# umautobots/LONER

Measured on AMD Instinct MI355X. Metric: training rays/sec, higher is better.
Workload: dtype f32

## Files before the change

### loner_amd/csrc/lnr_table_reduce.hip

```cpp
#include "lnr_density_api.h"
#include <cstdlib>

#define LNR_SLAB_GROUPS 16
__device__ __forceinline__ void slab_fold_block(const float* __restrict__ slabs, int n_slabs, int n_mlp, float* __restrict__ grad, int overwrite, int block) {
    __shared__ float part[LNR_SLAB_GROUPS][64];
    const int px = threadIdx.x & 63, gy = threadIdx.x >> 6;
    const int i = block * 64 + px;
    const int per = (n_slabs + LNR_SLAB_GROUPS - 1) / LNR_SLAB_GROUPS;
    int b = gy * per;
    const int b_end = min(n_slabs, b + per);
    float s0 = 0.0f, s1 = 0.0f, s2 = 0.0f, s3 = 0.0f;
    if (i < n_mlp) {
        for (; b + 3 < b_end; b += 4) {
            s0 += slabs[(size_t)b * n_mlp + i]; s1 += slabs[(size_t)(b + 1) * n_mlp + i];
            s2 += slabs[(size_t)(b + 2) * n_mlp + i]; s3 += slabs[(size_t)(b + 3) * n_mlp + i];
        }
        for (; b < b_end; ++b) s0 += slabs[(size_t)b * n_mlp + i];
    }
    part[gy][px] = (s0 + s1) + (s2 + s3);
    __syncthreads();
    if (gy == 0 && i < n_mlp) {
        float s = 0.0f;
#pragma unroll
        for (int k = 0; k < LNR_SLAB_GROUPS; ++k) s += part[k][px];
        grad[i] = overwrite ? s : grad[i] + s;
    }
}
__global__ void __launch_bounds__(64 * LNR_SLAB_GROUPS)
reduce_slabs_kernel(const float* __restrict__ slabs, int n_slabs, int n_mlp, float* __restrict__ grad, int overwrite) {
    slab_fold_block(slabs, n_slabs, n_mlp, grad, overwrite, (int)blockIdx.x);
}

template <int PAIR>
__device__ __forceinline__ void reduce_one(long long* acc, uint2 r, uint32_t base) {
    if (PAIR) {
        uint32_t pi; float v0, v1;
        lnr_unpack_pair(r, pi, v0, v1);
        unsigned long long* a = reinterpret_cast<unsigned long long*>(acc) + 2 * pi;
        if (__builtin_expect(__builtin_fmaxf(__builtin_fabsf(v0), __builtin_fabsf(v1)) < 256.0f, 1)) {
            atomicAdd(a, (unsigned long long)lnr_to_fix_small(v0));
            atomicAdd(a + 1, (unsigned long long)lnr_to_fix_small(v1));
        } else {
            atomicAdd(a, (unsigned long long)lnr_to_fix(v0));
            atomicAdd(a + 1, (unsigned long long)lnr_to_fix(v1));
        }
    } else {
        const float v = __uint_as_float(r.y);
        if (v != 0.0f) atomicAdd(reinterpret_cast<unsigned long long*>(&acc[r.x - base]), (unsigned long long)lnr_to_fix(v));
    }
}
__device__ __forceinline__ void reduce_xpair(long long* acc, const LnrXRec& r) {
    uint32_t pi, t; float a0, a1, fx;
    lnr_unpack_xpair(r, pi, t, a0, a1, fx);
    const uint32_t pj = pi ^ ((2u << t) - 1u);
    long long q[4];
    lnr_xpair_fix(a0, a1, fx, q);
    unsigned long long* a = reinterpret_cast<unsigned long long*>(acc);
    atomicAdd(a + 2 * pi, (unsigned long long)q[0]);
    atomicAdd(a + 2 * pi + 1, (unsigned long long)q[1]);
    atomicAdd(a + 2 * pj, (unsigned long long)q[2]);
    atomicAdd(a + 2 * pj + 1, (unsigned long long)q[3]);
}

#ifdef LNR_PHASE_TIMING
__device__ unsigned long long lnr_reduce_phase_cycles[LNR_N_PHASES];
#endif
#define RED_SLICE (1 << LNR_SLICE_SHIFT)

typedef uint32_t red_u32x3 __attribute__((ext_vector_type(3), aligned(4)));
typedef uint32_t red_u32x4 __attribute__((ext_vector_type(4)));
__device__ __forceinline__ LnrXRec load_xrec_stream(const char* p) {
    const red_u32x3 v = __builtin_nontemporal_load(reinterpret_cast<const red_u32x3*>(p));
    LnrXRec r; r.a = v.x; r.b = v.y; r.c = v.z;
    return r;
}
__device__ __forceinline__ uint4 load_rec2_stream(const uint4* p) {
    const red_u32x4 v = __builtin_nontemporal_load(reinterpret_cast<const red_u32x4*>(p));
    return make_uint4(v.x, v.y, v.z, v.w);
}

template <int PAIR, int RED_U>
__device__ __forceinline__ void reduce_regions(long long* acc, const int* __restrict__ wave_counts, const char* __restrict__ wave_regions, int n_regions,
                                               uint32_t region_bytes, bool xp, uint32_t base, int lane) {
    for (int r0 = 0; r0 < n_regions; r0 += 64) {
        const int nq = min(64, n_regions - r0);
        const int my_n = lane < nq ? wave_counts[r0 + lane] : 0;
        const char* round_regions = wave_regions + (size_t)r0 * region_bytes;
        if (xp) {
            LnrXRec cur[RED_U][2], nxt[RED_U][2];
            auto loadx = [&](int q0, LnrXRec out[RED_U][2]) {
#pragma unroll
                for (int u = 0; u < RED_U; ++u) {
                    const int q = q0 + u < nq ? q0 + u : nq - 1;
                    const int n = __builtin_amdgcn_readlane(my_n, q);
                    const char* rg = round_regions + (size_t)q * region_bytes;
                    out[u][0] = load_xrec_stream(rg + (lane < n ? lane : 0) * 12);
                    out[u][1] = load_xrec_stream(rg + (lane + 64 < n ? lane + 64 : 0) * 12);
                }
            };
            loadx(0, nxt);
            for (int q0 = 0; q0 < nq; q0 += RED_U) {
#pragma unroll
                for (int u = 0; u < RED_U; ++u) { cur[u][0] = nxt[u][0]; cur[u][1] = nxt[u][1]; }
                if (q0 + RED_U < nq) loadx(q0 + RED_U, nxt);
#pragma unroll
                for (int u = 0; u < RED_U; ++u) {
                    const int n = q0 + u < nq ? __builtin_amdgcn_readlane(my_n, q0 + u < 64 ? q0 + u : 63) : 0;
                    if (lane < n) reduce_xpair(acc, cur[u][0]);
                    if (lane + 64 < n) reduce_xpair(acc, cur[u][1]);
                }
            }
            unsigned long long more = __ballot(my_n > 128);
            while (more) {
                const int q = __builtin_ctzll(more);
                more &= more - 1ull;
                const int n = __builtin_amdgcn_readlane(my_n, q);
                const char* rg = round_regions + (size_t)q * region_bytes;
                for (int off = 128; off < n; off += 64 * 4) {
                    LnrXRec r[4];
#pragma unroll
                    for (int u = 0; u < 4; ++u) { const int k = off + 64 * u + lane; r[u] = load_xrec_stream(rg + (size_t)(k < n ? k : n - 1) * 12); }
#pragma unroll
                    for (int u = 0; u < 4; ++u) if (off + 64 * u + lane < n) reduce_xpair(acc, r[u]);
                }
            }
            continue;
        }
        uint4 cur[RED_U], nxt[RED_U];
        auto load4 = [&](int q0, uint4 out[RED_U]) {
#pragma unroll
            for (int u = 0; u < RED_U; ++u) {
                const int q = q0 + u < nq ? q0 + u : nq - 1;
                const int n = __builtin_amdgcn_readlane(my_n, q);
                out[u] = load_rec2_stream(reinterpret_cast<const uint4*>(round_regions + (size_t)q * region_bytes) + (2 * lane < n ? lane : 0));
            }
        };
        load4(0, nxt);
        for (int q0 = 0; q0 < nq; q0 += RED_U) {
#pragma unroll
            for (int u = 0; u < RED_U; ++u) cur[u] = nxt[u];
            if (q0 + RED_U < nq) load4(q0 + RED_U, nxt);
#pragma unroll
            for (int u = 0; u < RED_U; ++u) {
                const int n = q0 + u < nq ? __builtin_amdgcn_readlane(my_n, q0 + u < 64 ? q0 + u : 63) : 0;
                if (2 * lane < n) reduce_one<PAIR>(acc, make_uint2(cur[u].x, cur[u].y), base);
                if (2 * lane + 1 < n) reduce_one<PAIR>(acc, make_uint2(cur[u].z, cur[u].w), base);
            }
        }
        unsigned long long more = __ballot(my_n > 128);
        while (more) {
            const int q = __builtin_ctzll(more);
            more &= more - 1ull;
            const int n = __builtin_amdgcn_readlane(my_n, q);
            const uint2* rg = reinterpret_cast<const uint2*>(round_regions + (size_t)q * region_bytes);
            for (int off = 128; off < n; off += 128 * 4) {
                uint4 r[4];
#pragma unroll
                for (int u = 0; u < 4; ++u) { const int k = off + 128 * u + 2 * lane; r[u] = load_rec2_stream(reinterpret_cast<const uint4*>(rg) + (k < n ? k : 0) / 2); }
#pragma unroll
                for (int u = 0; u < 4; ++u) {
                    const int k = off + 128 * u + 2 * lane;
                    if (k < n) reduce_one<PAIR>(acc, make_uint2(r[u].x, r[u].y), base);
                    if (k + 1 < n) reduce_one<PAIR>(acc, make_uint2(r[u].z, r[u].w), base);
                }
            }
        }
    }
}

struct RedLevel { uint64_t lo, hi; };
__device__ __forceinline__ RedLevel red_level(const LnrNetSpec& spec, int l) {
    RedLevel r;
    r.lo = (uint64_t)spec.level_offset[l] * spec.n_features;
    r.hi = r.lo + (uint64_t)spec.level_size[l] * spec.n_features;
    return r;
}

template <int PAIR, int RED_U, int MINW>
__global__ void __launch_bounds__(1024, MINW)
table_grad_reduce_split_kernel(const LnrNetSpec spec, const void* __restrict__ regions_v, const RegionPlan plan, const int* __restrict__ counts, int bpg,
                               int maxo, long long* __restrict__ ovf) {
    extern __shared__ long long acc[];
    constexpr int slice = RED_SLICE, shift = LNR_SLICE_SHIFT;
    int b = blockIdx.x, l = 0, span = 0;
    int64_t my_ovf = 0;
    RedLevel lv;
    for (;; ++l) {
        lv = red_level(spec, l);
        span = (int)(((lv.hi - 1) >> shift) - (lv.lo >> shift)) + 1;
        const int n = plan.split[l] > 1 ? span * plan.split[l] : 0;
        if (b < n) break;
        b -= n;
        my_ovf += (int64_t)(lv.hi - lv.lo);
    }
    const int parts = plan.split[l], local = b / parts, part = b % parts;
    const uint32_t base = ((uint32_t)(lv.lo >> shift) + (uint32_t)local) << shift;
    const uint32_t region_bytes = plan.bytes[l];
    if (region_bytes == 0u) return;
#pragma unroll
    for (int i = threadIdx.x; i < slice; i += 1024) acc[i] = 0ll;
    __syncthreads();
    const int lane = threadIdx.x & 63, wave = __builtin_amdgcn_readfirstlane(threadIdx.x >> 6);
    const int per_part = (bpg + parts - 1) / parts, part_first = part * per_part, part_n = min(per_part, bpg - part_first);
    const int per_wave = (part_n + 15) / 16, first = part_first + wave * per_wave, n_regions = min(per_wave, part_first + part_n - first);
    if (n_regions > 0)
        reduce_regions<PAIR, RED_U>(acc, counts + ((size_t)l * maxo + local) * bpg + first,
                                    reinterpret_cast<const char*>(regions_v) + plan.off[l] + ((size_t)local * bpg + first) * (size_t)region_bytes, n_regions,
                                    region_bytes, PAIR && plan.xp[l] != 0, base, lane);
    __syncthreads();
#pragma unroll
    for (int k = 0; k < slice / 1024; ++k) {
        const int i = threadIdx.x + k * 1024;
        const uint64_t gi = (uint64_t)base + i;
        const long long q = acc[i];
        if (q != 0ll && gi >= lv.lo && gi < lv.hi) atomicAdd(reinterpret_cast<unsigned long long*>(ovf + my_ovf + (int64_t)(gi - lv.lo)), (unsigned long long)q);
    }
}

template <int PAIR, int RED_U, int MINW>
__global__ void __launch_bounds__(1024, MINW)
table_grad_reduce2_kernel(const LnrNetSpec spec, const void* __restrict__ regions_v, const RegionPlan plan, const int* __restrict__ counts, int bpg,
                          int maxo, long long* __restrict__ ovf, const int* __restrict__ ovf_flag, int epoch, float* __restrict__ grad_table,
                          int64_t n_table_floats, int overwrite, const float* __restrict__ slabs, int n_slabs, int n_mlp, float* __restrict__ grad_mlp) {
    extern __shared__ long long acc[];
    const int slab_blocks = slabs != nullptr ? (n_mlp + 63) / 64 : 0;
    const int owner_blocks = (int)gridDim.x - slab_blocks;
    if ((int)blockIdx.x >= owner_blocks) {
        slab_fold_block(slabs, n_slabs, n_mlp, grad_mlp, overwrite, (int)blockIdx.x - owner_blocks);
        return;
    }
    const int o = owner_blocks - 1 - (int)blockIdx.x;
    constexpr int slice = RED_SLICE, shift = LNR_SLICE_SHIFT;
    const uint32_t base = (uint32_t)o << shift;
    PHASE_INIT();
#pragma unroll
    for (int i = threadIdx.x; i < slice; i += 1024) acc[i] = 0ll;
    __syncthreads();
    PHASE(0);
    const int lane = threadIdx.x & 63, wave = __builtin_amdgcn_readfirstlane(threadIdx.x >> 6);
    constexpr int nwaves = 16;
    int64_t ovf_off = 0;
    for (int l = 0; l < spec.n_levels; ++l) {
        const RedLevel lv = red_level(spec, l);
        const uint64_t lo = lv.lo, hi = lv.hi;
        const int64_t my_ovf = ovf_off;
        ovf_off += (int64_t)(hi - lo);
        if (hi <= base || lo >= (uint64_t)base + slice) continue;
        if (plan.split[l] > 1 || ovf_flag[l] == epoch) {
            long long v[slice / 1024];
#pragma unroll
            for (int k = 0; k < slice / 1024; ++k) {
                const uint64_t gi = (uint64_t)base + threadIdx.x + k * 1024;
                v[k] = (gi >= lo && gi < hi) ? ovf[my_ovf + (int64_t)(gi - lo)] : 0ll;
            }
#pragma unroll
            for (int k = 0; k < slice / 1024; ++k) {
                if (v[k] != 0ll) {
                    acc[threadIdx.x + k * 1024] += v[k];
                    ovf[my_ovf + (int64_t)((uint64_t)base + threadIdx.x + k * 1024 - lo)] = 0ll;
                }
            }
            __syncthreads();
            PHASE(1);
        }
        const int local = o - (int)(lo >> shift);
        if (local < 0 || local >= maxo) continue;
        const uint32_t region_bytes = plan.bytes[l];
        if (region_bytes == 0u || plan.split[l] > 1) continue;
        const int per_wave = (bpg + nwaves - 1) / nwaves;
        const int first = wave * per_wave;
        const int n_regions = min(per_wave, bpg - first);
        if (n_regions > 0)
            reduce_regions<PAIR, RED_U>(acc, counts + ((size_t)l * maxo + local) * bpg + first,
                                        reinterpret_cast<const char*>(regions_v) + plan.off[l] + ((size_t)local * bpg + first) * (size_t)region_bytes, n_regions,
                                        region_bytes, PAIR && plan.xp[l] != 0, base, lane);
        PHASE(3);
    }
    __syncthreads();
    PHASE(5);
    {
        float g[slice / 1024];
#pragma unroll
        for (int k = 0; k < slice / 1024; ++k) {
            const int64_t gi = (int64_t)base + threadIdx.x + k * 1024;
            g[k] = (!overwrite && gi < n_table_floats) ? grad_table[gi] : 0.0f;
        }
#pragma unroll
        for (int k = 0; k < slice / 1024; ++k) {
            const int64_t gi = (int64_t)base + threadIdx.x + k * 1024;
            const long long q = acc[threadIdx.x + k * 1024];
            if (gi < n_table_floats && (overwrite || q != 0ll)) grad_table[gi] = g[k] + (float)((double)q * (1.0 / (double)LNR_FIX_SCALE));
        }
    }
    PHASE(6);
    PHASE_FLUSH(lnr_reduce_phase_cycles, 0);
}

void lnr_launch_slab_fold(const SlabFold& f, int overwrite, hipStream_t st) {
    LnrProfScope prof("reduce_slabs", st);
    hipLaunchKernelGGL(reduce_slabs_kernel, dim3(lnr_div_up(f.n_mlp, 64)), dim3(64 * LNR_SLAB_GROUPS), 0, st, f.slabs, f.n_slabs, f.n_mlp, f.grad, overwrite);
}

template <int PAIR, int U, int W>
static int launch_reduce_variant(const LnrNetSpec* spec, const TableGradSink& c, int n_owners, int n_split, const SlabFold& f, int overwrite, hipStream_t st) {
    const size_t lds = (size_t)RED_SLICE * sizeof(long long);
    if (hipFuncSetAttribute(reinterpret_cast<const void*>(table_grad_reduce2_kernel<PAIR, U, W>), hipFuncAttributeMaxDynamicSharedMemorySize, (int)lds) != hipSuccess ||
        hipFuncSetAttribute(reinterpret_cast<const void*>(table_grad_reduce_split_kernel<PAIR, U, W>), hipFuncAttributeMaxDynamicSharedMemorySize, (int)lds) != hipSuccess) {
        lnr_set_error("lnr_density_backward: hipFuncSetAttribute failed"); return LNR_ERR_LAUNCH;
    }
    if (n_split > 0) {
        LnrProfScope prof("table_grad_reduce_split", st);
        hipLaunchKernelGGL((table_grad_reduce_split_kernel<PAIR, U, W>), dim3(n_split), dim3(1024), lds, st, *spec, c.regions, c.plan, c.counts, c.bpg, c.maxo, c.ovf);
    }
    LnrProfScope prof("table_grad_reduce", st);
    const int slab_blocks = f.slabs != nullptr ? (f.n_mlp + 63) / 64 : 0;
    hipLaunchKernelGGL((table_grad_reduce2_kernel<PAIR, U, W>), dim3(n_owners + slab_blocks), dim3(1024), lds, st, *spec, c.regions, c.plan, c.counts, c.bpg, c.maxo,
                       c.ovf, c.ovf_flag, c.epoch, c.grad_table, spec->n_params - spec->n_mlp_params, overwrite, f.slabs, f.n_slabs, f.n_mlp, f.grad);
    return LNR_OK;
}
#ifndef LNR_RED_U
#define LNR_RED_U 2
#endif
#ifndef LNR_RED_W
#define LNR_RED_W 8
#endif
int lnr_launch_table_reduce(const LnrNetSpec* spec, const TableGradSink& sink, int n_owners, int n_split, const SlabFold& fold, int overwrite, hipStream_t st) {
    if (spec->n_features < 2) return launch_reduce_variant<0, LNR_RED_U, LNR_RED_W>(spec, sink, n_owners, n_split, fold, overwrite, st);
    return launch_reduce_variant<1, LNR_RED_U, LNR_RED_W>(spec, sink, n_owners, n_split, fold, overwrite, st);
}

#ifdef LNR_PHASE_TIMING
void lnr_table_reduce_print_phases(hipStream_t st) {
    static const char* names[LNR_N_PHASES] = {"zero LDS", "overflow fold", "-", "records", "-", "final barrier", "write-out"};
    unsigned long long h[LNR_N_PHASES];
    if (getenv("LNR_PHASE_TIMING") && lnr_phase_fetch(HIP_SYMBOL(lnr_reduce_phase_cycles), h, LNR_N_PHASES, st)) lnr_phase_print("table_grad_reduce", names, h);
}
#endif
```

Before: 2.027 million.

## Balance table-grad reduction across waves with LDS atomic work claiming

Replaces the static per-wave split of regions in the table gradient reduce kernels with dynamic claiming: each wave atomically grabs small groups of regions from an LDS counter (one counter per level). This targets load imbalance when region counts are skewed across waves. The split kernel also exits early when its part has no entries, which skips zeroing and the writeback. The cost is extra LDS atomics and shared memory, plus a smaller batch of regions per claim round.

```diff
diff --git a/loner_amd/csrc/lnr_table_reduce.hip b/loner_amd/csrc/lnr_table_reduce.hip
--- a/loner_amd/csrc/lnr_table_reduce.hip
+++ b/loner_amd/csrc/lnr_table_reduce.hip
@@ -80,71 +80,30 @@
 }
 
 template <int PAIR, int RED_U>
-__device__ __forceinline__ void reduce_regions(long long* acc, const int* __restrict__ wave_counts, const char* __restrict__ wave_regions, int n_regions,
-                                               uint32_t region_bytes, bool xp, uint32_t base, int lane) {
-    for (int r0 = 0; r0 < n_regions; r0 += 64) {
-        const int nq = min(64, n_regions - r0);
-        const int my_n = lane < nq ? wave_counts[r0 + lane] : 0;
-        const char* round_regions = wave_regions + (size_t)r0 * region_bytes;
-        if (xp) {
-            LnrXRec cur[RED_U][2], nxt[RED_U][2];
-            auto loadx = [&](int q0, LnrXRec out[RED_U][2]) {
-#pragma unroll
-                for (int u = 0; u < RED_U; ++u) {
-                    const int q = q0 + u < nq ? q0 + u : nq - 1;
-                    const int n = __builtin_amdgcn_readlane(my_n, q);
-                    const char* rg = round_regions + (size_t)q * region_bytes;
-                    out[u][0] = load_xrec_stream(rg + (lane < n ? lane : 0) * 12);
-                    out[u][1] = load_xrec_stream(rg + (lane + 64 < n ? lane + 64 : 0) * 12);
-                }
-            };
-            loadx(0, nxt);
-            for (int q0 = 0; q0 < nq; q0 += RED_U) {
-#pragma unroll
-                for (int u = 0; u < RED_U; ++u) { cur[u][0] = nxt[u][0]; cur[u][1] = nxt[u][1]; }
-                if (q0 + RED_U < nq) loadx(q0 + RED_U, nxt);
-#pragma unroll
-                for (int u = 0; u < RED_U; ++u) {
-                    const int n = q0 + u < nq ? __builtin_amdgcn_readlane(my_n, q0 + u < 64 ? q0 + u : 63) : 0;
-                    if (lane < n) reduce_xpair(acc, cur[u][0]);
-                    if (lane + 64 < n) reduce_xpair(acc, cur[u][1]);
-                }
-            }
-            unsigned long long more = __ballot(my_n > 128);
-            while (more) {
-                const int q = __builtin_ctzll(more);
-                more &= more - 1ull;
-                const int n = __builtin_amdgcn_readlane(my_n, q);
-                const char* rg = round_regions + (size_t)q * region_bytes;
-                for (int off = 128; off < n; off += 64 * 4) {
-                    LnrXRec r[4];
-#pragma unroll
-                    for (int u = 0; u < 4; ++u) { const int k = off + 64 * u + lane; r[u] = load_xrec_stream(rg + (size_t)(k < n ? k : n - 1) * 12); }
-#pragma unroll
-                    for (int u = 0; u < 4; ++u) if (off + 64 * u + lane < n) reduce_xpair(acc, r[u]);
-                }
-            }
-            continue;
-        }
-        uint4 cur[RED_U], nxt[RED_U];
-        auto load4 = [&](int q0, uint4 out[RED_U]) {
+__device__ __forceinline__ void reduce_regions(long long* acc, int my_n, const char* __restrict__ round_regions, int nq, uint32_t region_bytes, bool xp,
+                                               uint32_t base, int lane) {
+    if (xp) {
+        LnrXRec cur[RED_U][2], nxt[RED_U][2];
+        auto loadx = [&](int q0, LnrXRec out[RED_U][2]) {
 #pragma unroll
             for (int u = 0; u < RED_U; ++u) {
                 const int q = q0 + u < nq ? q0 + u : nq - 1;
                 const int n = __builtin_amdgcn_readlane(my_n, q);
-                out[u] = load_rec2_stream(reinterpret_cast<const uint4*>(round_regions + (size_t)q * region_bytes) + (2 * lane < n ? lane : 0));
+                const char* rg = round_regions + (size_t)q * region_bytes;
+                out[u][0] = load_xrec_stream(rg + (lane < n ? lane : 0) * 12);
+                out[u][1] = load_xrec_stream(rg + (lane + 64 < n ? lane + 64 : 0) * 12);
             }
         };
-        load4(0, nxt);
+        loadx(0, nxt);
         for (int q0 = 0; q0 < nq; q0 += RED_U) {
 #pragma unroll
-            for (int u = 0; u < RED_U; ++u) cur[u] = nxt[u];
-            if (q0 + RED_U < nq) load4(q0 + RED_U, nxt);
+            for (int u = 0; u < RED_U; ++u) { cur[u][0] = nxt[u][0]; cur[u][1] = nxt[u][1]; }
+            if (q0 + RED_U < nq) loadx(q0 + RED_U, nxt);
 #pragma unroll
             for (int u = 0; u < RED_U; ++u) {
                 const int n = q0 + u < nq ? __builtin_amdgcn_readlane(my_n, q0 + u < 64 ? q0 + u : 63) : 0;
-                if (2 * lane < n) reduce_one<PAIR>(acc, make_uint2(cur[u].x, cur[u].y), base);
-                if (2 * lane + 1 < n) reduce_one<PAIR>(acc, make_uint2(cur[u].z, cur[u].w), base);
+                if (lane < n) reduce_xpair(acc, cur[u][0]);
+                if (lane + 64 < n) reduce_xpair(acc, cur[u][1]);
             }
         }
         unsigned long long more = __ballot(my_n > 128);
@@ -152,20 +111,74 @@
             const int q = __builtin_ctzll(more);
             more &= more - 1ull;
             const int n = __builtin_amdgcn_readlane(my_n, q);
-            const uint2* rg = reinterpret_cast<const uint2*>(round_regions + (size_t)q * region_bytes);
-            for (int off = 128; off < n; off += 128 * 4) {
-                uint4 r[4];
-#pragma unroll
-                for (int u = 0; u < 4; ++u) { const int k = off + 128 * u + 2 * lane; r[u] = load_rec2_stream(reinterpret_cast<const uint4*>(rg) + (k < n ? k : 0) / 2); }
-#pragma unroll
-                for (int u = 0; u < 4; ++u) {
-                    const int k = off + 128 * u + 2 * lane;
-                    if (k < n) reduce_one<PAIR>(acc, make_uint2(r[u].x, r[u].y), base);
-                    if (k + 1 < n) reduce_one<PAIR>(acc, make_uint2(r[u].z, r[u].w), base);
-                }
-            }
-        }
-    }
+            const char* rg = round_regions + (size_t)q * region_bytes;
+            for (int off = 128; off < n; off += 64 * 4) {
+                LnrXRec r[4];
+#pragma unroll
+                for (int u = 0; u < 4; ++u) { const int k = off + 64 * u + lane; r[u] = load_xrec_stream(rg + (size_t)(k < n ? k : n - 1) * 12); }
+#pragma unroll
+                for (int u = 0; u < 4; ++u) if (off + 64 * u + lane < n) reduce_xpair(acc, r[u]);
+            }
+        }
+        return;
+    }
+    uint4 cur[RED_U], nxt[RED_U];
+    auto load4 = [&](int q0, uint4 out[RED_U]) {
+#pragma unroll
+        for (int u = 0; u < RED_U; ++u) {
+            const int q = q0 + u < nq ? q0 + u : nq - 1;
+            const int n = __builtin_amdgcn_readlane(my_n, q);
+            out[u] = load_rec2_stream(reinterpret_cast<const uint4*>(round_regions + (size_t)q * region_bytes) + (2 * lane < n ? lane : 0));
+        }
+    };
+    load4(0, nxt);
+    for (int q0 = 0; q0 < nq; q0 += RED_U) {
+#pragma unroll
+        for (int u = 0; u < RED_U; ++u) cur[u] = nxt[u];
+        if (q0 + RED_U < nq) load4(q0 + RED_U, nxt);
+#pragma unroll
+        for (int u = 0; u < RED_U; ++u) {
+            const int n = q0 + u < nq ? __builtin_amdgcn_readlane(my_n, q0 + u < 64 ? q0 + u : 63) : 0;
+            if (2 * lane < n) reduce_one<PAIR>(acc, make_uint2(cur[u].x, cur[u].y), base);
+            if (2 * lane + 1 < n) reduce_one<PAIR>(acc, make_uint2(cur[u].z, cur[u].w), base);
+        }
+    }
+    unsigned long long more = __ballot(my_n > 128);
+    while (more) {
+        const int q = __builtin_ctzll(more);
+        more &= more - 1ull;
+        const int n = __builtin_amdgcn_readlane(my_n, q);
+        const uint2* rg = reinterpret_cast<const uint2*>(round_regions + (size_t)q * region_bytes);
+        for (int off = 128; off < n; off += 128 * 4) {
+            uint4 r[4];
+#pragma unroll
+            for (int u = 0; u < 4; ++u) { const int k = off + 128 * u + 2 * lane; r[u] = load_rec2_stream(reinterpret_cast<const uint4*>(rg) + (k < n ? k : 0) / 2); }
+#pragma unroll
+            for (int u = 0; u < 4; ++u) {
+                const int k = off + 128 * u + 2 * lane;
+                if (k < n) reduce_one<PAIR>(acc, make_uint2(r[u].x, r[u].y), base);
+                if (k + 1 < n) reduce_one<PAIR>(acc, make_uint2(r[u].z, r[u].w), base);
+            }
+        }
+    }
+}
+
+#ifndef LNR_RED_CLAIM
+#define LNR_RED_CLAIM 4
+#endif
+static_assert(LNR_RED_CLAIM >= 2 && LNR_RED_CLAIM <= 64, "a claim is one round of reduce_regions: lane q holds region q's count");
+template <int PAIR, int RED_U>
+__device__ __forceinline__ void reduce_claimed(long long* acc, int* counter, const int* __restrict__ counts, const char* __restrict__ regions, int n_regions,
+                                               uint32_t region_bytes, bool xp, uint32_t base, int lane) {
+    const int group = max(RED_U, min(LNR_RED_CLAIM, n_regions >> 5));
+    auto claim = [&]() {
+        int first = 0;
+        if (lane == 0) first = atomicAdd(counter, group);
+        return __builtin_amdgcn_readfirstlane(first);
+    };
+    auto count_of = [&](int first) { return (lane < group && first + lane < n_regions) ? counts[first + lane] : 0; };
+    for (int first = claim(); first < n_regions; first = claim())
+        reduce_regions<PAIR, RED_U>(acc, count_of(first), regions + (size_t)first * region_bytes, min(group, n_regions - first), region_bytes, xp, base, lane);
 }
 
 struct RedLevel { uint64_t lo, hi; };
@@ -197,15 +210,21 @@
     const uint32_t base = ((uint32_t)(lv.lo >> shift) + (uint32_t)local) << shift;
     const uint32_t region_bytes = plan.bytes[l];
     if (region_bytes == 0u) return;
+    int* claim = reinterpret_cast<int*>(acc + slice);
+    const int lane = threadIdx.x & 63;
+    const int per_part = (bpg + parts - 1) / parts, part_first = part * per_part, part_n = min(per_part, bpg - part_first);
+    {
+        int any = 0;
+        for (int i = threadIdx.x; i < part_n; i += 1024) any |= counts[((size_t)l * maxo + local) * bpg + part_first + i];
+        if (!__syncthreads_or(any)) return;
+    }
 #pragma unroll
     for (int i = threadIdx.x; i < slice; i += 1024) acc[i] = 0ll;
-    __syncthreads();
-    const int lane = threadIdx.x & 63, wave = __builtin_amdgcn_readfirstlane(threadIdx.x >> 6);
-    const int per_part = (bpg + parts - 1) / parts, part_first = part * per_part, part_n = min(per_part, bpg - part_first);
-    const int per_wave = (part_n + 15) / 16, first = part_first + wave * per_wave, n_regions = min(per_wave, part_first + part_n - first);
-    if (n_regions > 0)
-        reduce_regions<PAIR, RED_U>(acc, counts + ((size_t)l * maxo + local) * bpg + first,
-                                    reinterpret_cast<const char*>(regions_v) + plan.off[l] + ((size_t)local * bpg + first) * (size_t)region_bytes, n_regions,
+    if (threadIdx.x == 0) claim[0] = 0;
+    __syncthreads();
+    if (part_n > 0)
+        reduce_claimed<PAIR, RED_U>(acc, claim, counts + ((size_t)l * maxo + local) * bpg + part_first,
+                                    reinterpret_cast<const char*>(regions_v) + plan.off[l] + ((size_t)local * bpg + part_first) * (size_t)region_bytes, part_n,
                                     region_bytes, PAIR && plan.xp[l] != 0, base, lane);
     __syncthreads();
 #pragma unroll
@@ -233,12 +252,13 @@
     constexpr int slice = RED_SLICE, shift = LNR_SLICE_SHIFT;
     const uint32_t base = (uint32_t)o << shift;
     PHASE_INIT();
+    int* claim = reinterpret_cast<int*>(acc + slice);
 #pragma unroll
     for (int i = threadIdx.x; i < slice; i += 1024) acc[i] = 0ll;
+    if (threadIdx.x < LNR_MAX_LEVELS) claim[threadIdx.x] = 0;
     __syncthreads();
     PHASE(0);
-    const int lane = threadIdx.x & 63, wave = __builtin_amdgcn_readfirstlane(threadIdx.x >> 6);
-    constexpr int nwaves = 16;
+    const int lane = threadIdx.x & 63;
     int64_t ovf_off = 0;
     for (int l = 0; l < spec.n_levels; ++l) {
         const RedLevel lv = red_level(spec, l);
@@ -267,13 +287,9 @@
         if (local < 0 || local >= maxo) continue;
         const uint32_t region_bytes = plan.bytes[l];
         if (region_bytes == 0u || plan.split[l] > 1) continue;
-        const int per_wave = (bpg + nwaves - 1) / nwaves;
-        const int first = wave * per_wave;
-        const int n_regions = min(per_wave, bpg - first);
-        if (n_regions > 0)
-            reduce_regions<PAIR, RED_U>(acc, counts + ((size_t)l * maxo + local) * bpg + first,
-                                        reinterpret_cast<const char*>(regions_v) + plan.off[l] + ((size_t)local * bpg + first) * (size_t)region_bytes, n_regions,
-                                        region_bytes, PAIR && plan.xp[l] != 0, base, lane);
+        reduce_claimed<PAIR, RED_U>(acc, claim + l, counts + ((size_t)l * maxo + local) * bpg,
+                                    reinterpret_cast<const char*>(regions_v) + plan.off[l] + (size_t)local * bpg * (size_t)region_bytes, bpg,
+                                    region_bytes, PAIR && plan.xp[l] != 0, base, lane);
         PHASE(3);
     }
     __syncthreads();
@@ -303,7 +319,7 @@
 
 template <int PAIR, int U, int W>
 static int launch_reduce_variant(const LnrNetSpec* spec, const TableGradSink& c, int n_owners, int n_split, const SlabFold& f, int overwrite, hipStream_t st) {
-    const size_t lds = (size_t)RED_SLICE * sizeof(long long);
+    const size_t lds = (size_t)RED_SLICE * sizeof(long long) + LNR_MAX_LEVELS * sizeof(int);
     if (hipFuncSetAttribute(reinterpret_cast<const void*>(table_grad_reduce2_kernel<PAIR, U, W>), hipFuncAttributeMaxDynamicSharedMemorySize, (int)lds) != hipSuccess ||
         hipFuncSetAttribute(reinterpret_cast<const void*>(table_grad_reduce_split_kernel<PAIR, U, W>), hipFuncAttributeMaxDynamicSharedMemorySize, (int)lds) != hipSuccess) {
         lnr_set_error("lnr_density_backward: hipFuncSetAttribute failed"); return LNR_ERR_LAUNCH;
```

Result: no change. 2.043 million, median of 6 (+0.8%).
